# armadaproject/armada

Measured on NVIDIA H100. Metric: job-placements/sec per scheduling round; 100k nodes x 1M jobs, higher is better.
Workload: dtype int64+f64

## Files before the change

armada_b200/csrc/armada_dev.h:

```cpp
#pragma once
#include <stdint.h>
#ifndef ARMADA_EMU
#include <vector_types.h>
#endif

#include "armada_b200.h"

#define ARMADA_DEV_MAX_QUEUES 128
#define ARMADA_DEV_MAX_SLOTS 22
#define ARMADA_DEV_VARIANTS (1 + ARMADA_MAX_AWAY)

enum StatSlot {
  STAT_ITERS = 0,
  STAT_PROBES = 1,
  STAT_PLACEMENTS = 2,
  STAT_FAIR = 3,
  STAT_RESCANS = 4,
  STAT_KERNEL = 5,
  STAT_STARTUP = 6,
  STAT_RUNS = 7,
  STAT_PROF = 8,
  STAT_PROF_PQ_TOP = 8,
  STAT_PROF_GANG = 9,
  STAT_PROF_SELECT = 10,
  STAT_PROF_BIND = 11,
  STAT_BATCH_ITERS = 12,
  STAT_PROF_RESULT = 13,
  STAT_PROF_ADVANCE = 14,
  STAT_PROF_CLEAR = 15,
  STAT_BT_CYC = 16,
  STAT_BT_BUILD = 16,
  STAT_BT_HORIZON = 17,
  STAT_BT_RANK = 18,
  STAT_BT_WAIT = 19,
  STAT_BT_COMMIT = 20,
  STAT_BT_CONTROL = 21,
  STAT_BT_BATCHES = 22,
  STAT_BT_EPILOGUE = 23,
  STAT_BT_DBG = 24,
  STAT_CHAIN_BUSY = 24,
  STAT_CHAIN_WAIT = 25,
  STAT_PIPELINE_RUNS = 26,
  STAT_BT_CUT = 27,
  STAT_SLOW_STEPS = 28,
  STAT_SLOW_CYCLES = 29,
  STAT_REFILLS = 30,
  STAT_REFILL_CYCLES = 31,
  STAT_TL_PRECREATE = 32,
  STAT_TL_FIRST_BATCH_WAIT = 33,
  STAT_TL_AFTER_CHAIN_WAIT = 34,
  STAT_TL_FAILED_ITERS = 35,
  STAT_TL_FAILED_CYCLES = 36,
  STAT_TL_FAIR_QUERY = 37,
  STAT_TL_LEVEL_SCAN = 38,
  STAT_TL_EVICTED_REBIND = 39,
  STAT_GL_WAIT_INDEX = 40,
  STAT_GL_RING_FULL = 41,
  STAT_GL_SELECT_QUEUED = 42,
  STAT_GL_BIND_QUEUED = 43,
  STAT_GL_FAIR_VICTIMS = 44,
  STAT_GL_PROLOGUE = 45,
  STAT_GL_SELECT_COUNT = 46,
  STAT_GATE_RUN = 47,
  STAT_GATE_SKIPPED = 48,
  STAT_BT_FAILS = 49,
  STAT_COUNT = 50,
};

enum CountSlot {
  CNT_SCHED_JOBS = 0,
  CNT_SCHED_GANGS = 1,
  CNT_EVICTED_JOBS = 2,
  CNT_TERMINATION = 3,
  CNT_GLOBAL_TOKENS = 4,
  CNT_ERROR = 5,
  CNT_COUNT = 8,
};
#define ARMADA_DEV_E_DEADLINE 100

struct DevCfg {
  int32_t D, R, PL, PC, Q, C, T, S, rows;
  uint32_t N, J, G;
  int32_t indexed_resource[ARMADA_MAX_RESOURCES];
  int64_t res_scale[ARMADA_MAX_RESOURCES];
  int32_t key_shift[ARMADA_MAX_RESOURCES];
  int32_t res_key_shift[ARMADA_MAX_RESOURCES];
  int32_t res_key_width[ARMADA_MAX_RESOURCES];
  int32_t node_bits;
  int32_t key_total_bits;
  int32_t key_width[ARMADA_MAX_RESOURCES];
  unsigned long long key_guard;
  int32_t swar_ok;
  int32_t cls_global;
  int32_t exact;
  int64_t index_res[ARMADA_MAX_RESOURCES];
  int32_t collect_excl;
  int32_t k32_ok;
  int32_t min_bind_prio;
  int32_t priorities[ARMADA_MAX_PRIORITIES];
  ArmadaPriorityClass pcs[ARMADA_MAX_PRIORITY_CLASSES];
  int64_t total_resources[ARMADA_MAX_RESOURCES];
  double drf_mult[ARMADA_MAX_RESOURCES];
  int64_t max_to_schedule[ARMADA_MAX_RESOURCES];
  uint8_t has_round_limit, protect_uncapped, prefer_large, disable_home, disable_away, disable_gang_away,
      global_inf, _pad;
  double protected_fraction;
  uint32_t max_lookback, disallowed_mask;
  double global_tokens;
  int64_t global_burst;
  int32_t max_slots, sw, tw;
  int32_t win_w;
  uint32_t off_cls, off_win, off_touched, off_slot, off_skey, off_srow, off_ssc, off_sgpos, off_hb_key, off_hb_row, off_hb_sc,
      off_ring, off_bt_k0, off_bt_k1, off_bt_id;
  int32_t bt_wq;
  int32_t bt_np;
  uint32_t uni_V;
  uint32_t floating_mask;
  int32_t floating_configured;
  int64_t floating_limit[ARMADA_MAX_RESOURCES];
// ... 54 lines not shown
  const int64_t* queue_burst;
  const uint8_t* queue_inf;
  int64_t* alloc;
  uint32_t* bound_node;
  uint8_t* evicted_on_node;
  int32_t* sched_prio;
  uint8_t* q_successful;
  uint8_t* q_unsuccessful;
  uint8_t* q_rescheduled;
  uint8_t* q_evicted;
  uint8_t* q_reason;
  uint8_t* jc_evicted;
  uint32_t* jc_card;
  uint32_t* assigned_node;
  uint8_t* in_preempted;
  uint8_t* in_scheduled;
  uint8_t* in_sae;
  uint8_t* ev_mark;
  uint8_t* gang_ev;
  uint8_t* has_pctx;
  uint32_t* res_node;
  int32_t* res_sched_at;
  int32_t* res_preempted_at;
  uint8_t* res_method;
  uint32_t* res_seq;
  uint32_t* fp_seq;
  uint8_t* fp_flags;
  uint32_t* gang_fill;
  uint32_t* gang_buf;
  int32_t* ev_index_of_job;
  uint32_t* ev_job_by_index;
  uint8_t* ev_alive;
  uint32_t* evq_start;
  uint32_t* evq_jobs;
  uint64_t* sort_keys;
  uint64_t* sort_keys2;
  uint32_t* sort_vals;
  uint32_t* sort_vals2;
  uint32_t* counters;
  uint8_t* unfeasible;
  unsigned long long* g0;
  unsigned long long* g0_tmp;
  uint32_t* g0_sc;
  uint32_t* bt_job;
  uint32_t* bt_cls;
  uint32_t* bt_pos;
  uint32_t* bt_rank;
  uint2* bt_seq;
  int64_t* bt_asum;
  uint32_t* bt_card;
  uint4* bt_item;
  uint32_t* bt_gnode;
  uint32_t* gang_bak;
  const uint32_t* gang_uni_label;
  const uint32_t* uni_start;
  const uint32_t* class_uni_row;
  const uint8_t* gang_simple;
  uint32_t* excl;
  const uint32_t* row_type_excl;
  UndoRec* undo_log;
  uint32_t* fp_head;
  uint32_t* fp_next;
  uint32_t* nl_start;
  uint2* nl_item;
  uint32_t* nl_pos;
  uint32_t* nver;
  uint32_t* fc_ver;
  uint32_t* bver;
  uint32_t* fc_bver;
  unsigned long long* fc_bmax;
  int64_t* q_alloc;
  int64_t* q_alloc_pc;
  double* q_fair;
  double* q_tokens;
  int64_t* s_scheduled;
  int64_t* s_evicted;
  int64_t* s_counts;
  uint32_t* dbg_host;
  unsigned long long* stats;
};
```

armada_b200/csrc/armada_host.inc:

```

#define CUDA_TRY(expr)                                                                     \
  do {                                                                                     \
    cudaError_t _e = (expr);                                                               \
    if (_e != cudaSuccess) {                                                               \
      g_last_error = std::string(#expr) + ": " + cudaGetErrorString(_e);                   \
      return ARMADA_E_CUDA;                                                                \
    }                                                                                      \
  } while (0)

#ifdef ARMADA_EMU
static std::recursive_mutex& emu_mutex() {
  static std::recursive_mutex m;
  return m;
}
#define ARMADA_EMU_SERIAL std::lock_guard<std::recursive_mutex> emu_lock_(emu_mutex())
#else
#define ARMADA_EMU_SERIAL ((void)0)
#endif

template <class T>
struct PinnedVec {
  T* p = nullptr;
  size_t n = 0, cap = 0;
  PinnedVec() = default;
// ... 1045 lines not shown
  DA(P.alloc, (size_t)PL * D * N);
  DA(P.xkey, cfg.exact ? (size_t)PL * N : 1);
  DA(P.cls_glob, cfg.cls_global ? sizeof(ClassRec) * (size_t)C : 16);
  DA(P.bound_node, J);
  DA(P.evicted_on_node, J);
  DA(P.sched_prio, J);
  DA(P.q_successful, J);
  DA(P.q_unsuccessful, J);
  DA(P.q_rescheduled, J);
  DA(P.q_evicted, J);
  DA(P.q_reason, J);
  DA(P.jc_evicted, J);
  DA(P.jc_card, J);
  DA(P.assigned_node, J);
  DA(P.in_preempted, J);
  DA(P.in_scheduled, J);
  DA(P.in_sae, J);
  DA(P.ev_mark, J);
  DA(P.gang_ev, G);
  DA(P.has_pctx, J);
  DA(P.res_node, J);
  DA(P.res_sched_at, J);
  DA(P.res_preempted_at, J);
  DA(P.res_method, J);
  DA(P.res_seq, J);
  DA(P.fp_seq, J);
  DA(P.fp_flags, 4 * (size_t)J);
  DA(P.gang_fill, G);
  DA(P.gang_buf, h.gang_off[G]);
  DA(P.ev_index_of_job, J);
  DA(P.ev_job_by_index, J);
  DA(P.ev_alive, J);
  DA(P.evq_start, Q + 1);
  DA(P.evq_jobs, J);
  DA(P.sort_keys, J);
  DA(P.sort_keys2, J);
  DA(P.sort_vals, std::max(J, N));
  DA(P.sort_vals2, std::max(J, N));
  DA(P.counters, 16);
  DA(P.unfeasible, C);
  DA(P.g0, N);
  DA(P.g0_tmp, N);
  P.g0_sc = (uint32_t*)P.g0_tmp;
  DA(P.bt_job, 2 * (size_t)Q * 64);
  DA(P.bt_cls, 2 * (size_t)Q * 64);
  DA(P.bt_pos, 2 * (size_t)Q * 64);
  DA(P.bt_rank, 2 * (size_t)Q * 64);
  DA(P.bt_seq, 2 * (size_t)Q * 64);
  DA(P.bt_asum, 2 * (size_t)Q * ARMADA_MAX_RESOURCES);
  DA(P.bt_card, 2 * (size_t)Q * 64);
  DA(P.bt_item, 2 * (size_t)Q * 64);
  DA(P.bt_gnode, 2 * (size_t)Q * 64 * 64);
  DA(P.gang_bak, 32 * (4 + ARMADA_MAX_RESOURCES * 2));
  DA(P.excl, cfg.collect_excl ? (size_t)J * ARMADA_EXCLUDED_KINDS : 16);
  DA(P.undo_log, 3 * (size_t)J + 16);
  DA(P.ev_rec, J);
  DA(P.fp_head, N);
  DA(P.fp_next, J);
  DA(P.nl_start, (size_t)N + 1);
  DA(P.nl_item, J);
  DA(P.nl_pos, J);
  DA(P.nver, N);
  DA(P.fc_ver, 16 * (size_t)N);
  DA(P.bver, (N + 255) / 256 + 1);
  DA(P.fc_bver, 8 * ((size_t)(N + 255) / 256 + 1));
  DA(P.fc_bmax, 8 * ((size_t)(N + 255) / 256 + 1));
  DA(P.q_alloc, (size_t)Q * D);
  DA(P.q_alloc_pc, (size_t)Q * PC * D);
  DA(P.q_fair, (size_t)Q * 3);
  DA(P.q_tokens, Q);
  DA(P.s_scheduled, D);
  DA(P.s_evicted, D);
  DA(P.s_counts, CNT_COUNT);
  DA(P.stats, STAT_COUNT);
  {
    void* dp = nullptr;
    CUDA_TRY(cudaHostGetDevicePointer(&dp, r->h_dbg, 0));
    P.dbg_host = (uint32_t*)dp;
  }
  DA(r->d_state, J);
  DA(r->d_method, J);
  DA(r->d_reason, J);
  DA(r->d_node, J);
  DA(r->d_sched_at, J);
  DA(r->d_preempted_at, J);
  DA(r->d_evict_queue, Q);
  DA(r->d_oversub, N);
  DA(r->d_hist, 256 * (size_t)grid_for(std::max<uint32_t>(std::max(J, N), 1), RS_THREADS * RS_ITEMS) + 1024);
  if (!in->queue_allocated_by_pc || !in->queue_constrained_demand) {
    int64_t* d_demand_pc = nullptr;
    DA(d_demand_pc, (size_t)Q * PC * D);
    CUDA_TRY(cudaMemsetAsync(d_demand_pc, 0, (size_t)Q * PC * D * sizeof(int64_t), r->stream));
    ARMADA_LAUNCH(k_snapshot_jobs, grid_for(std::max<uint32_t>(J, 1)), 256, 0, r->stream, cfg, P, const_cast<int64_t*>(P.queue_alloc_pc0), d_demand_pc,
                  in->queue_allocated_by_pc ? 0 : 1);
    if (!in->queue_constrained_demand) {
      ARMADA_LAUNCH(k_snapshot_queues, grid_for((size_t)Q * D, 128), 128, 0, r->stream, cfg, P, d_demand_pc, const_cast<int64_t*>(P.queue_cdemand));
    }
    CUDA_TRY(cudaGetLastError());
  }
#undef DA
  CUDA_TRY(cudaStreamSynchronize(r->stream));
  return ARMADA_OK;
}
#undef UNSUP
#undef PINNED
}
// ... 234 lines not shown
  const ArmadaRound::Snapshot& h = r->snap;
  if (!r->uploaded || !h.valid) return fail_status(ARMADA_E_STATE, "armada_round_download_snapshot without armada_round_upload_cluster");
  auto out = [](auto* dst, const auto& src) {
    if (dst) std::copy(src.begin(), src.end(), dst);
  };
  out(node_state, h.state);
  out(node_allocatable, h.alloc);
  out(node_static_class, h.sclass);
  out(total_resources, h.total);
  out(max_resources_to_schedule, h.max_to_schedule);
  out(queue_limit, h.queue_limit);
  return ARMADA_OK;
}

#define ROUND_LAUNCH(r, kern, grid, block, smem, ...) \
  do { ARMADA_LAUNCH(kern, grid, block, smem, (r)->stream, __VA_ARGS__); ++(r)->launches; } while (0)

static void radix_sort(ArmadaRound* r, uint32_t n, const std::vector<int>& shifts, unsigned long long*& keys, unsigned long long*& keys_tmp,
                       uint32_t*& vals, uint32_t*& vals_tmp) {
  const uint32_t blocks = grid_for(n, RS_THREADS * RS_ITEMS);
  for (int shift : shifts) {
    ROUND_LAUNCH(r, k_rs_hist, blocks, RS_THREADS, 0, keys, n, shift, r->d_hist);
    ROUND_LAUNCH(r, k_rs_scan, 1, 1024, 0, r->d_hist, 256 * blocks);
    ROUND_LAUNCH(r, k_rs_scatter, blocks, RS_THREADS, 0, keys, vals, keys_tmp, vals_tmp, n, shift, r->d_hist);
    std::swap(keys, keys_tmp);
    std::swap(vals, vals_tmp);
  }
}

static int32_t sort_evicted(ArmadaRound* r, uint32_t n) {
  DevCfg& c = r->cfg;
  DevPtrs& P = r->P;
  unsigned long long *k0 = (unsigned long long*)P.sort_keys, *k1 = (unsigned long long*)P.sort_keys2;
  uint32_t *v0 = P.sort_vals, *v1 = P.sort_vals2;
  if (n > 0) {
    int rank_bytes = (bits_for(c.J > 1 ? c.J - 1 : 1) + 7) / 8;
    std::vector<int> shifts;
    for (int b = 0; b < rank_bytes; ++b) shifts.push_back(8 * b);
    int queue_bytes = (bits_for(c.Q > 1 ? (uint32_t)c.Q - 1 : 1) + 7) / 8;
    for (int b = 0; b < queue_bytes; ++b) shifts.push_back(32 + 8 * b);
    radix_sort(r, n, shifts, k0, k1, v0, v1);
    ROUND_LAUNCH(r, k_copy_u32, grid_for(n), 256, 0, P.evq_jobs, v0, n);
    ROUND_LAUNCH(r, k_build_ev_records, grid_for(n), 256, 0, c, P, n);
  }
  ROUND_LAUNCH(r, k_evq_bounds, grid_for((size_t)c.Q + 1, 128), 128, 0, c, P, k0, n);
  CUDA_TRY(cudaGetLastError());
  return ARMADA_OK;
}

static int32_t sort_g0(ArmadaRound* r) {
  DevCfg& c = r->cfg;
  DevPtrs& P = r->P;
  const uint32_t n = c.N;
  ROUND_LAUNCH(r, k_g0_keys, grid_for(n), 256, 0, c, P);
  unsigned long long *k0 = P.g0, *k1 = P.g0_tmp;
  uint32_t *v0 = P.sort_vals, *v1 = P.sort_vals2;
  std::vector<int> shifts;
  for (int shift = 0; shift < r->key_bits; shift += 8) shifts.push_back(shift);
  radix_sort(r, n, shifts, k0, k1, v0, v1);
  if (shifts.size() & 1) {
    CUDA_TRY(cudaMemcpyAsync(P.g0, P.g0_tmp, (size_t)n * sizeof(unsigned long long), cudaMemcpyDeviceToDevice, r->stream));
  }
  ROUND_LAUNCH(r, k_g0_sc, grid_for(n), 256, 0, c, P);
#ifdef ARMADA_EMU
  if (getenv("EMU_DUMP_G0")) {
    fprintf(stderr, "g0 (N=%u node_bits=%d key_bits=%d shifts", n, c.node_bits, r->key_bits);
    for (int i = 0; i < c.R; ++i) fprintf(stderr, " %d", c.key_shift[i]);
    fprintf(stderr, "):");
    for (uint32_t i = 0; i < n; ++i) fprintf(stderr, " %llx", P.g0[i]);
    fprintf(stderr, "\n");
  }
#endif
  CUDA_TRY(cudaGetLastError());
  return ARMADA_OK;
}

static void launch_xkeys(ArmadaRound* r) { ROUND_LAUNCH(r, k_xkeys, grid_for((size_t)r->cfg.PL * r->cfg.N), 256, 0, r->cfg, r->P); }

static int32_t run_reset_bind(ArmadaRound* r) {
  DevCfg& c = r->cfg;
  if (c.collect_excl) CUDA_TRY(cudaMemsetAsync(r->P.excl, 0, (size_t)c.J * ARMADA_EXCLUDED_KINDS * sizeof(uint32_t), r->stream));
  ROUND_LAUNCH(r, k_reset, r->num_sms * 4, 256, 0, c, r->P);
  ROUND_LAUNCH(r, k_bind_running, grid_for(std::max<uint32_t>(c.J, 1)), 256, 0, c, r->P);
  ROUND_LAUNCH(r, k_queue_init, 1, 32, 0, c, r->P);
  return ARMADA_OK;
}

static int32_t run_evict(ArmadaRound* r, int pass, uint32_t* evicted) {
  DevCfg& c = r->cfg;
  DevPtrs& P = r->P;
  const uint32_t gj = grid_for(std::max<uint32_t>(c.J, 1)), gg = grid_for(std::max<uint32_t>(c.G, 1));
  if (pass == 1) {
    ROUND_LAUNCH(r, k_evict_queue_flags, grid_for(c.Q, 128), 128, 0, c, P, r->d_evict_queue);
    ROUND_LAUNCH(r, k_evict_balance, gj, 256, 0, c, P, r->d_evict_queue);
  } else {
    CUDA_TRY(cudaMemsetAsync(P.counters, 0, sizeof(uint32_t), r->stream));
    ROUND_LAUNCH(r, k_oversub_mask, grid_for(c.N), 256, 0, c, P, r->d_oversub);
    ROUND_LAUNCH(r, k_evict_oversub, gj, 256, 0, c, P, r->d_oversub);
  }
  ROUND_LAUNCH(r, k_evict_gangs, gj, 256, 0, c, P);
  ROUND_LAUNCH(r, k_evict_account, gj, 256, 0, c, P, pass);
  ROUND_LAUNCH(r, k_clear_gang_ev, gg, 256, 0, c, P);
  CUDA_TRY(cudaMemcpyAsync(evicted, P.counters, sizeof(uint32_t), cudaMemcpyDeviceToHost, r->stream));
  CUDA_TRY(cudaStreamSynchronize(r->stream));
  return ARMADA_OK;
}
// ... 9 lines not shown
  a.with_queued = pass == 1;
  a.skip_key_check = pass == 2;
  a.consider_priority = pass == 2;
  a.assign_indices = pass == 2 || num_evicted > 0;
  a.pass = pass;
  a.num_evicted = num_evicted;
  a.budget_ns = budget_ns;
  a.g0_valid = pass == 1 && !r->cfg.exact;
  const PassKernel kern = pass_kernel(r->cfg.D);
  CUDA_TRY(cudaEventRecord(r->evp[2 * pass - 2], r->stream));
  ROUND_LAUNCH(r, kern, 1, PASS_THREADS, r->smem_bytes, r->cfg, r->P, a);
  CUDA_TRY(cudaEventRecord(r->evp[2 * pass - 1], r->stream));
  return ARMADA_OK;
}

static int32_t snapshot_first_pass(ArmadaRound* r) {
  DevPtrs& P = r->P;
  cudaStream_t s = r->stream;
  const size_t Jn = r->cfg.J;
  CUDA_TRY(cudaMemcpyAsync(P.fp_seq, P.res_seq, Jn * sizeof(uint32_t), cudaMemcpyDeviceToDevice, s));
  const uint8_t* flags[4] = {P.q_successful, P.q_rescheduled, P.q_unsuccessful, P.q_reason};
  for (int k = 0; k < 4; ++k) CUDA_TRY(cudaMemcpyAsync(P.fp_flags + k * Jn, flags[k], Jn, cudaMemcpyDeviceToDevice, s));
  return ARMADA_OK;
}

static int32_t run_finalize(ArmadaRound* r) {
  ROUND_LAUNCH(r, k_finalize, grid_for(std::max<uint32_t>(r->cfg.J, 1)), 256, 0, r->cfg, r->P, r->d_state, r->d_node, r->d_sched_at,
               r->d_preempted_at, r->d_method, r->d_reason);
  CUDA_TRY(cudaEventRecord(r->ev1, r->stream));
  CUDA_TRY(cudaGetLastError());
  cudaError_t e = cudaStreamSynchronize(r->stream);
  if (e != cudaSuccess) {
    g_last_error = std::string("cudaStreamSynchronize: ") + cudaGetErrorString(e) + watchdog_report(r->h_dbg);
    return ARMADA_E_CUDA;
  }
  return ARMADA_OK;
}

static int32_t read_stats(ArmadaRound* r, uint32_t e1, uint32_t e2) {
  long long counts[CNT_COUNT];
  unsigned long long dstats[STAT_COUNT];
  CUDA_TRY(cudaMemcpy(counts, r->P.s_counts, sizeof(counts), cudaMemcpyDeviceToHost));
  CUDA_TRY(cudaMemcpy(dstats, r->P.stats, sizeof(dstats), cudaMemcpyDeviceToHost));
  if (counts[CNT_ERROR] == ARMADA_DEV_E_DEADLINE)
    return fail_status(ARMADA_E_DEADLINE, "the round did not finish within its time budget; nothing was committed");
  if (counts[CNT_ERROR] != 0) return fail_status(ARMADA_E_INTERNAL, "device invariant violated, code " + std::to_string(counts[CNT_ERROR]));
  float ms = 0;
  CUDA_TRY(cudaEventElapsedTime(&ms, r->ev0, r->ev1));
  r->stats = ArmadaRoundStats{};
  if (getenv("ARMADA_PRINT_STATS"))
    fprintf(stderr,
            "armada stats: kernel_cycles=%llu startup=%llu pipeline_runs=%llu chain_busy=%llu chain_wait=%llu epilogue=%llu precreate=%llu first_batch_wait=%llu "
            "after_chain_wait=%llu failed_iters=%llu failed_cycles=%llu fair_query_cycles=%llu level_scan_cycles=%llu evicted_rebind_cycles=%llu "
            "gate_scans=%llu gate_skips=%llu bt_fails=%llu\n",
            dstats[STAT_KERNEL], dstats[STAT_STARTUP], dstats[STAT_RUNS], dstats[STAT_CHAIN_BUSY], dstats[STAT_CHAIN_WAIT], dstats[STAT_BT_EPILOGUE],
            dstats[STAT_TL_PRECREATE], dstats[STAT_TL_FIRST_BATCH_WAIT], dstats[STAT_TL_AFTER_CHAIN_WAIT], dstats[STAT_TL_FAILED_ITERS],
            dstats[STAT_TL_FAILED_CYCLES], dstats[STAT_TL_FAIR_QUERY], dstats[STAT_TL_LEVEL_SCAN], dstats[STAT_TL_EVICTED_REBIND],
            dstats[STAT_GATE_RUN], dstats[STAT_GATE_SKIPPED], dstats[STAT_BT_FAILS]);
  if (getenv("ARMADA_PRINT_STATS"))
    fprintf(stderr,
            "armada general loop: wait_index_warps=%llu ring_full=%llu select_queued=%llu (n=%llu) bind_queued=%llu fair_victims=%llu iteration_prologue=%llu\n",
            dstats[STAT_GL_WAIT_INDEX], dstats[STAT_GL_RING_FULL], dstats[STAT_GL_SELECT_QUEUED], dstats[STAT_GL_SELECT_COUNT],
            dstats[STAT_GL_BIND_QUEUED], dstats[STAT_GL_FAIR_VICTIMS], dstats[STAT_GL_PROLOGUE]);
  r->stats.loop_iterations = dstats[STAT_ITERS];
  r->stats.probes = dstats[STAT_PROBES];
  r->stats.placements = dstats[STAT_PLACEMENTS];
  r->stats.fair_preemption_scans = dstats[STAT_FAIR];
  r->stats.tree_rescans = dstats[STAT_RESCANS];
  for (int i = 0; i < 8; ++i) r->stats.phase_cycles[i] = dstats[STAT_PROF + i];
  for (int i = 0; i < 8; ++i) r->stats.batch_cycles[i] = dstats[STAT_BT_CYC + i];
  for (int i = 0; i < 8; ++i) r->stats.batch_debug[i] = dstats[STAT_BT_DBG + i];
  r->stats.evicted_pass1 = e1;
  r->stats.evicted_pass2 = e2;
  r->stats.gpu_launches = r->launches;
  r->stats.device_ms = ms;
  float p1 = 0, p2 = 0;
  CUDA_TRY(cudaEventElapsedTime(&p1, r->evp[0], r->evp[1]));
  if (e2 > 0) CUDA_TRY(cudaEventElapsedTime(&p2, r->evp[2], r->evp[3]));
  r->stats.schedule_pass_ms = p1 + p2;
  return ARMADA_OK;
}

int32_t armada_round_run(ArmadaRound* r, ArmadaRoundStats* stats) { return armada_round_run_deadline(r, stats, 0); }

int32_t armada_round_run_deadline(ArmadaRound* r, ArmadaRoundStats* stats, uint64_t budget_ns) {
  if (!r) return fail_status(ARMADA_E_INVALID, "null handle");
  const auto t_run0 = std::chrono::steady_clock::now();
  auto budget_left = [&]() -> unsigned long long {
    if (!budget_ns) return 0ull;
    const uint64_t used = (uint64_t)std::chrono::duration_cast<std::chrono::nanoseconds>(std::chrono::steady_clock::now() - t_run0).count();
    return used >= budget_ns ? 1ull : (unsigned long long)(budget_ns - used);
  };
  if (!r->uploaded) return fail_status(ARMADA_E_STATE, "armada_round_run before armada_round_upload");
  ARMADA_EMU_SERIAL;
  CUDA_TRY(cudaSetDevice(r->device));
  r->launches = 0;
  CUDA_TRY(cudaEventRecord(r->ev0, r->stream));
  int32_t st;
  uint32_t e1 = 0, e2 = 0;
  if ((st = run_reset_bind(r)) || (st = run_evict(r, 1, &e1)) || (st = sort_evicted(r, e1))) return st;
  const unsigned long long budget1 = budget_left();
  if ((st = build_index(r, 1)) || (st = run_pass(r, 1, e1, budget1)) || (st = snapshot_first_pass(r))) return st;
  if ((st = run_evict(r, 2, &e2))) return st;
  if (e2 > 0) {
    if ((st = sort_evicted(r, e2))) return st;
    const unsigned long long budget2 = budget_left();
    if ((st = build_index(r, 2)) || (st = run_pass(r, 2, e2, budget2))) return st;
  }
  if ((st = run_finalize(r)) || (st = read_stats(r, e1, e2))) return st;
  if (stats) *stats = r->stats;
  r->ran = true;
// ... 374 lines not shown
```

armada_b200/csrc/armada_pass.inc:

```

#define g_c (H->env_c)
#define g_p (H->env_p)
#define g_a (H->env_a)

#define PASS_WARPS 16
#define PASS_THREADS (PASS_WARPS * 32)
#define IDX_WARPS 15
#define CTL_WARP (PASS_WARPS - 1)
#define IDX_OWNERS (IDX_WARPS - 1)
#define WIN 32
#define WIN_TARGET 12
#define WIN_LOW 4
#define MSG_CAP 32
#define TLOG_CAP 32

enum { MSG_EXIT = 0, MSG_UPDATE0 = 1, MSG_NEWSLOT = 2, MSG_SCAN = 3, MSG_BATCH = 4, MSG_SUCC = 5, MSG_FAIR = 6 };
#define BT_RING 32

#define REC_EVICTED 0x80000000u
#define REC_GANG 0x40000000u
#define REC_QEV 0x20000000u
#define REC_GS 0x10000000u
#define REC_GSL 0x08000000u
#define REC_CLS_MASK 0x00FFFFFFu
// ... 3013 lines not shown
#pragma unroll
    for (int t = 0; t < ARMADA_DEV_MAX_SLOTS; ++t) Df[t] = 0;
    const unsigned long long G = g_c.key_guard;
    const uint32_t okm = H->slot_okp;
    uint32_t seen = 0;
    for (uint32_t pos = (uint32_t)w * 32u + (uint32_t)l; pos < g_c.N; pos += IDX_WARPS * 32u) {
      const unsigned long long gk = g_p.g0[pos];
      const uint32_t n = (uint32_t)(gk & nodemask);
      if ((V.touched[n >> 5] >> (n & 31)) & 1u) continue;
      if ((gk >> g_c.key_total_bits) != 0) continue;
      const uint32_t sc = g_p.g0_sc[pos];
      uint32_t m = 0;
#pragma unroll
      for (int t = 0; t < ARMADA_DEV_MAX_SLOTS; ++t)
        if (t < ns) {
          const SlotHdr& sh = V.slot[t];
          const bool f = sh.active && ((okm >> t) & 1u) && Idx<DMAX>::slot_static(sh, sc) && ((((gk | G) - H->slot_preq[t]) & G) == G);
          m |= (f ? 1u : 0u) << t;
        }
#pragma unroll
      for (int t = 0; t < ARMADA_DEV_MAX_SLOTS; ++t) Df[t] |= ((m >> t) & 1u) ? ~m : m;
      uint32_t fresh = m & ~seen;
      seen |= m;
      while (fresh) {
        const int t = __ffs(fresh) - 1;
        fresh &= fresh - 1;
        atomicMin(&H->grp_first[t], pos);
      }
    }
#pragma unroll
    for (int t = 0; t < ARMADA_DEV_MAX_SLOTS; ++t)
      if (t < ns) {
        const uint32_t r = __reduce_or_sync(FULL, Df[t]);
        if (l == 0 && r) atomicOr(&H->grp_diff[t], r);
      }
    __threadfence_block();
    bar_idx();
    if (w == 0) {
      if (l < ns && V.slot[l].active) {
        uint32_t leader = (uint32_t)l;
        for (int t = 0; t < l; ++t)
          if (V.slot[t].active && V.slot[t].row == V.slot[l].row && !((H->grp_diff[l] >> t) & 1u)) {
            leader = (uint32_t)t;
            break;
          }
        H->grp_of[l] = leader;
      }
      if (l == 0) H->grp_ns = ns;
    }
    __threadfence_block();
    bar_idx();
  }

  static __device__ ARMADA_NOINLINE void fill_lazy(int w, bool have_first) {
    const int ns = H->num_slots;
    if (w < IDX_OWNERS)
      for (int s = w; s < ns; s += IDX_OWNERS) {
        SlotHdr& sh = V.slot[s];
        if (!sh.active || !sh.lazy) continue;
        const uint32_t first = have_first ? H->grp_first[s] : 0u;
        __syncwarp();
        if (lane_id() == 0) {
          if (have_first && sh.cursor < first) {
            const uint32_t c = first < g_c.N ? first : g_c.N;
            sh.cursor = c;
            sh.wm = c < g_c.N ? g_p.g0[c] : KEY_INF;
          }
          sh.lazy = 0;
        }
        __syncwarp();
        Idx<DMAX>::ensure_head(s, true);
      }
    __threadfence_block();
    bar_idx();
  }

  static __device__ ARMADA_NOINLINE void table_build() {
    const int l = lane_id();
    const int ns = H->num_slots;
    const uint32_t ltm = (1u << l) - 1u;
    bool valid = false;
    uint32_t node = NONE;
    bool ok = true;
    BtRes* T = H->bt_ring;
    for (int s = 0; s < ns && ok; ++s) {
      const SlotHdr& sh = V.slot[s];
      if (!sh.active) continue;
      if (sh.lostmin != KEY_INF) ok = false;
      const uint32_t cnt = sh.cnt;
      const bool tch = (uint32_t)l < cnt && V.sgpos[s * WIN + l] == NONE;
      const uint32_t nid = tch ? (uint32_t)(V.skey[s * WIN + l] & nodemask) : NONE;
      if (!__ballot_sync(FULL, tch)) continue;
      bool dupe = false;
#pragma unroll
      for (int j = 0; j < 32; ++j) {
        const uint32_t nj = __shfl_sync(FULL, node, j);
        dupe = dupe || (tch && nj == nid);
      }
      const uint32_t newm = __ballot_sync(FULL, tch && !dupe);
      if (!newm) continue;
      const uint32_t freem = ~__ballot_sync(FULL, valid);
      const int nnew = __popc(newm);
      if (nnew > __popc(freem)) {
        ok = false;
        break;
      }
// ... 369 lines not shown
    return 1;
  }

  static __device__ __forceinline__ uint32_t warp_min_u32(uint32_t v) {
#ifdef ARMADA_EMU
    return __reduce_min_sync(FULL, v);
#else
    uint32_t m;
    asm volatile("redux.sync.min.u32 %0, %1, 0xffffffff;" : "=r"(m) : "r"(v));
    return m;
#endif
  }
  template <bool K32, class KT>
  static __device__ __forceinline__ int place(Lane<K32>& X, uint32_t& have, const uint32_t exh, const uint32_t lead, const KT Gk, const uint4 r, uint4* recp) {
    bool win, cand;
    uint32_t sbit;
    if (K32) {
      sbit = r.y;
      const uint32_t d = (uint32_t)X.Y - r.x;
      const bool fit = ((d & (uint32_t)Gk) == (uint32_t)Gk) && (X.mystat & sbit);
      const uint32_t m = warp_min_u32(fit ? X.ck : 0xFFFFFFFFu);
      if (m == 0xFFFFFFFFu) return 2;
      win = X.ck == m;
      cand = m & 1u;
      if (win) {
        X.Y = d;
        X.ck -= r.w;
        recp->w = X.node;
      }
    } else {
      sbit = r.w;
      const unsigned long long d = (unsigned long long)X.Y - (((unsigned long long)r.y << 32) | r.x);
      const bool fit = ((d & (unsigned long long)Gk) == (unsigned long long)Gk) && (X.mystat & sbit);
      const unsigned long long m = warp_min_u64(fit ? (unsigned long long)X.Y : KEY_INF);
      if (m == KEY_INF) return 2;
      win = (unsigned long long)X.Y == m;
      cand = m & 1ull;
      if (win) {
        X.Y = d;
        recp->w = X.node;
      }
    }
    if (cand) {
      if (win) {
        if (K32) X.ck &= ~1u;
        else X.Y &= ~(KT)1;
        X.mystat = X.fullstat;
        atomicOr(&V.touched[X.node >> 5], 1u << (X.node & 31));
      }
      have = exh | __reduce_or_sync(FULL, is_cand<K32>(X) ? X.mystat : 0u);
      if (~have & lead) return 3;
    }
    return 0;
  }
  template <bool K32, class KT>
  static __device__ __forceinline__ int place_pair(Lane<K32>& X, uint32_t& have, const uint32_t exh, const uint32_t lead, const KT Gk, uint4* const rec,
                                                   uint32_t& t, const uint32_t total) {
    const KT NOFIT = ~(KT)0;
    auto req_of = [](const uint4 r) -> KT { return K32 ? (KT)r.x : (KT)(((unsigned long long)r.y << 32) | r.x); };
    auto grp_of = [](const uint4 r) -> uint32_t { return K32 ? r.y : r.w; };
    auto wmin = [](const KT v) -> KT { return K32 ? (KT)warp_min_u32((uint32_t)v) : (KT)warp_min_u64((unsigned long long)v); };
    auto gfit = [Gk](const KT d) -> bool { return (~d & Gk) == 0; };
    auto row_won = [](const KT d) -> KT { return K32 ? d : (KT)(d & ~(KT)1); };
    uint4 ra = rec[t], rb = rec[t + 1];
    for (;;) {
      const uint32_t left = total - t;
      const uint4 ran = rec[t + 2];
      uint4 rbn = rb;
      if (left >= 2) rbn = rec[t + 3];
      const KT ck = K32 ? (KT)X.ck : X.Y;
      const uint32_t sw = ((K32 ? X.ck : (uint32_t)X.Y) & 1u) ? X.fullstat : X.mystat;
      const KT da = X.Y - req_of(ra), db = X.Y - req_of(rb);
      const KT Ya = row_won(da), cka = K32 ? (KT)((X.ck - ra.w) & ~1u) : Ya;
      const KT dab = Ya - req_of(rb);
      const KT ka = (X.mystat & grp_of(ra)) ? ck : NOFIT;
      const KT ma = wmin(gfit(da) ? ka : NOFIT);
      const KT kb0 = (gfit(db) && (X.mystat & grp_of(rb))) ? ck : NOFIT;
      const KT kb1 = (gfit(dab) && (sw & grp_of(rb))) ? cka : NOFIT;
      const bool wa = ck == ma;
      const KT mb = wmin(wa ? kb1 : kb0);
      if (ma == NOFIT) return 2;
      const KT cka_post = wa ? cka : ck;
      const KT Yb = wa ? row_won(dab) : row_won(db);
      const KT ckb = K32 ? (KT)(((uint32_t)cka_post - rb.w) & ~1u) : Yb;
      if (wa) {
        X.Y = Ya;
        if (K32) X.ck = (uint32_t)cka;
        X.mystat = sw;
        rec[t].w = X.node;
      }
      ++t;
      if (ma & 1u) {
        if (wa) atomicOr(&V.touched[X.node >> 5], 1u << (X.node & 31));
        have = exh | __reduce_or_sync(FULL, is_cand<K32>(X) ? X.mystat : 0u);
        if (~have & lead) return 3;
      }
      if (t == total) return 0;
      if (mb == NOFIT) return 2;
      const bool wb = cka_post == mb;
      if (wb) {
        X.Y = Yb;
        if (K32) X.ck = (uint32_t)ckb;
        X.mystat = sw;
        rec[t].w = X.node;
      }
      ++t;
      if (mb & 1u) {
        if (wb) atomicOr(&V.touched[X.node >> 5], 1u << (X.node & 31));
        have = exh | __reduce_or_sync(FULL, is_cand<K32>(X) ? X.mystat : 0u);
        if (~have & lead) return 3;
      }
      if (t == total) return 0;
      ra = ran;
      rb = rbn;
    }
  }
  template <bool K32, class KT>
  static __device__ __forceinline__ bool ensure_groups(Lane<K32>& X, uint32_t& have, uint32_t& exh, const uint32_t lead, int ns, const KT Gk) {
    uint32_t need = ~have & lead;
    while (need) {
      const uint32_t s = (uint32_t)(__ffs(need) - 1);
      int r = install_bulk<K32, KT>(X, have, s, ns, Gk);
      if (r == 0) {
        if (!window_refill(s)) {
          have |= 1u << s;
          exh |= 1u << s;
          r = 1;
        } else {
          r = install_bulk<K32, KT>(X, have, s, ns, Gk);
        }
      }
      if (r != 1 && !install_general<K32>(&X, &have, &exh, s, ns)) return false;
      need = ~have & lead;
    }
    return true;
  }

  static __device__ __forceinline__ void chain_wait_first() {
    SPIN_BEGIN;
    while (Idx<DMAX>::uniform_ld(&H->pl_ready) == 0) {
      Ctl<DMAX>::service_fence();
      SPIN_CHECK(20);
      armada_emu_yield();
    }
    __threadfence_block();
  }

  static __device__ __forceinline__ long long chain_wait_batch(uint32_t kb) {
    const long long tw0 = clock64();
    SPIN_BEGIN;
    while ((uint32_t)Idx<DMAX>::uniform_ld(&H->pl_ready) <= kb) {
      SPIN_CHECK(21);
      armada_emu_yield();
    }
    __threadfence_block();
    return clock64() - tw0;
  }

  static __device__ __forceinline__ void chain_hand_over(uint32_t kb, uint32_t t, uint32_t total, bool failed) {
    __threadfence_block();
    __syncwarp();
    if (lane_id() == 0) {
      H->bt_done[kb & 1u] = t;
// ... 572 lines not shown
#define BT_CLOCK(slot)                                  \
  do {                                                  \
    if (w == 0 && lane_id() == 0) {                     \
      long long _t = clock64();                         \
      H->stat[slot] += (unsigned long long)(_t - t0);   \
      t0 = _t;                                          \
    }                                                   \
  } while (0)
  static __device__ __forceinline__ void produce(int w, int b, bool first, long long& t0) {
    for (int q = w; q < g_c.Q; q += IDX_WARPS) batch_build(q, b, first);
    __threadfence_block();
    bar_idx();
    BT_CLOCK(STAT_BT_BUILD);
    if (w == 0) {
      batch_horizon(b);
      if (lane_id() == 0) H->pl_skip = first ? 0u : ld_vol(&H->pl_cut);
    }
    __threadfence_block();
    bar_idx();
    BT_CLOCK(STAT_BT_HORIZON);
    if (H->pl_skip) return;
    batch_rank(w, b);
    for (int q = w; q < g_c.Q; q += IDX_WARPS) batch_advance(q, b);
    __threadfence();
    bar_idx();
    BT_CLOCK(STAT_BT_RANK);
  }

  static __device__ ARMADA_NOINLINE void restart(int w, int b, long long& t0) {
    const uint4 tail = __ldcg(&g_p.bt_item[buf_of(b).goff + H->bt_done[b] - 1]);
    const uint2 job = __ldcg(&g_p.bt_seq[buf_of(b).goff + H->bt_done[b] - 1]);
    const int qf = (int)tail.x;
    for (int q = w; q < g_c.Q; q += IDX_WARPS)
      if (H->bt_repeek[q] && q != qf) Ctl<DMAX>::pq_update(q, true);
    __threadfence_block();
    bar_idx();
    if (w == 0) {
      Ctl<DMAX>::mark_unfeasible(job.y, ARMADA_REASON_JOB_DOES_NOT_FIT);
      Ctl<DMAX>::pq_update(qf, true);
      if (lane_id() < g_c.D) H->sp_sched[lane_id()] = H->s_scheduled[lane_id()];
      if (lane_id() == 0) st_vol(&H->pl_cut, 0u);
    }
    __threadfence_block();
    bar_idx();
    produce(w, b, true, t0);
  }

  static __device__ ARMADA_NOINLINE void batch_run(int w) {
    long long t0 = clock64();
    const int ns = H->num_slots;
    const bool regroup = g_c.swar_ok && H->grp_ns != ns;
    if (regroup) group_slots(w);
    fill_lazy(w, regroup);
    produce(w, 0, true, t0);
    if (w == 0) table_build();
    __threadfence_block();
    bar_idx();
    const bool run = H->bt_total[0] > 0;
    if (run && w < IDX_OWNERS)
      for (int s = w; s < ns; s += IDX_OWNERS)
        if (V.slot[s].active) win_strip(s, false);
    __threadfence_block();
    bar_idx();
    if (w == 0 && lane_id() == 0) st_vol(&H->pl_ready, 1u);
    uint32_t kb = 0;
    while (H->bt_total[kb & 1u] > 0) {
      const int b = (int)(kb & 1u);
      produce(w, b ^ 1, false, t0);
      if (w == 0 && lane_id() == 0) st_vol(&H->pl_ready, kb + 2u);
      {
        SPIN_BEGIN;
        while ((uint32_t)Idx<DMAX>::uniform_ld(&H->pl_chain) <= kb) {
          SPIN_CHECK(22);
          idle_pause();
        }
        __threadfence_block();
      }
      BT_CLOCK(STAT_BT_WAIT);
      apply_results(w, b);
      for (int q = w; q < g_c.Q; q += IDX_WARPS) batch_commit(q, b);
      __threadfence();
      bar_idx();
      if (w == 0 && lane_id() == 0) {
        H->pl_seq += H->bt_done[b];
        H->stat[STAT_BT_BATCHES] += 1;
        if (H->bt_done[b] < H->bt_total[b]) H->stat[STAT_BT_CUT] += 1;
      }
      BT_CLOCK(STAT_BT_COMMIT);
      if (H->bt_fail[b]) {
        restart(w, b, t0);
        if (w == 0 && lane_id() == 0) st_vol(&H->pl_ready, kb + 3u);
        kb += 2;
        continue;
      }
      if (H->bt_done[b] < H->bt_total[b]) break;
      ++kb;
    }
    {
      SPIN_BEGIN;
      while (Idx<DMAX>::uniform_ld(&H->pl_home) == 0) {
        SPIN_CHECK(23);
        idle_pause();
      }
      __threadfence_block();
    }
    if (run && w < IDX_OWNERS)
// ... 173 lines not shown
```

armada_b200/csrc/armada_round.cu:

```cuda
#ifdef ARMADA_EMU
#include "cuda_emu.h"
#else
#include <cuda_runtime.h>
#define ARMADA_LAUNCH(kern, grid, block, smem, stream, ...) kern<<<(grid), (block), (smem), (stream)>>>(__VA_ARGS__)
#define ARMADA_DYN_SMEM(name) extern __shared__ __align__(16) unsigned char name[]
#define ARMADA_NAMED_BARRIER(id, count) asm volatile("bar.sync %0, %1;" ::"n"(id), "n"(count) : "memory")
static __device__ __forceinline__ void armada_emu_yield() {}
#define ARMADA_NOINLINE __noinline__
#define ARMADA_EMU_MARK(id) ((void)0)
#define ARMADA_PREFETCH_L1(p) asm volatile("prefetch.global.L1 [%0];" ::"l"(p))
#endif

#include <algorithm>
#include <atomic>
#include <memory>
#include <condition_variable>
#include <mutex>
#include <chrono>
#include <thread>
#include <type_traits>
#include <cmath>
#include <cstdio>
#include <cstring>
#include <numeric>
// ... 321 lines not shown
    tmp[threadIdx.x] = v;
    __syncthreads();
    for (int off = 1; off < 1024; off <<= 1) {
      uint32_t t = threadIdx.x >= (unsigned)off ? tmp[threadIdx.x - off] : 0;
      __syncthreads();
      tmp[threadIdx.x] += t;
      __syncthreads();
    }
    uint32_t incl = tmp[threadIdx.x];
    if (i < len) hist[i] = carry + incl - v;
    __syncthreads();
    if (threadIdx.x == 1023) carry += incl;
    __syncthreads();
  }
}
__global__ void k_rs_scatter(const unsigned long long* keys, const uint32_t* vals, unsigned long long* keys_out,
                             uint32_t* vals_out, uint32_t n, int shift, const uint32_t* hist) {
  __shared__ unsigned long long sk[RS_THREADS * RS_ITEMS];
  __shared__ uint32_t sv[RS_THREADS * RS_ITEMS];
  size_t base = (size_t)blockIdx.x * RS_THREADS * RS_ITEMS;
  uint32_t cnt = 0;
  for (int i = 0; i < RS_ITEMS; ++i) {
    size_t k = base + (size_t)i * RS_THREADS + threadIdx.x;
    uint32_t li = i * RS_THREADS + threadIdx.x;
    if (k < n) {
      sk[li] = keys[k];
      sv[li] = vals[k];
    }
  }
  __syncthreads();
  uint32_t m = n - base < (size_t)RS_THREADS * RS_ITEMS ? (uint32_t)(n - base) : RS_THREADS * RS_ITEMS;
  uint32_t off = hist[(size_t)threadIdx.x * gridDim.x + blockIdx.x];
  for (uint32_t li = 0; li < m; ++li) {
    if (((sk[li] >> shift) & 255) == threadIdx.x) {
      keys_out[off + cnt] = sk[li];
      vals_out[off + cnt] = sv[li];
      ++cnt;
    }
  }
}

__global__ void k_g0_keys(DevCfg c, DevPtrs P) {
  size_t n = blockIdx.x * (size_t)blockDim.x + threadIdx.x;
  if (n >= c.N) return;
  unsigned long long key = n;
  bool neg = false;
  for (int i = 0; i < c.R; ++i) {
    int64_t v = P.alloc[(size_t)c.indexed_resource[i] * c.N + n];
    neg = neg || v < 0;
    key |= (unsigned long long)v << c.key_shift[i];
  }
  unsigned long long marker = 1ull << c.key_total_bits;
  P.g0[n] = neg ? (marker | n) : key;
}

__device__ __forceinline__ unsigned long long xfield_of(int64_t v, int64_t res) {
  if (v < 0) return 0ull;
  long long q = (long long)((double)v / (double)res);
  while (q * res > v) --q;
  while ((q + 1) * res <= v) ++q;
  return (unsigned long long)q + 1ull;
}
__global__ void k_xkeys(DevCfg c, DevPtrs P) {
  size_t i = blockIdx.x * (size_t)blockDim.x + threadIdx.x;
  if (i >= (size_t)c.PL * c.N) return;
  const size_t p = i / c.N, n = i - p * c.N;
  unsigned long long key = P.node_xrank[n];
  for (int k = 0; k < c.R; ++k)
    key |= xfield_of(P.alloc[(p * c.D + c.indexed_resource[k]) * c.N + n], c.index_res[k]) << c.key_shift[k];
  P.xkey[i] = key;
}

__global__ void k_snapshot_jobs(DevCfg c, DevPtrs P, int64_t* alloc_pc, int64_t* demand_pc, int want_alloc) {
  size_t j = blockIdx.x * (size_t)blockDim.x + threadIdx.x;
  if (j >= c.J) return;
  const uint32_t q = P.job_queue[j];
  if (q == NONE) return;
  const uint32_t cls = P.job_class[j];
  const uint32_t pc = P.class_pc[cls];
  const bool running = P.job_node0[j] != NONE;
  const bool cordoned = P.queue_cordoned[q] != 0;
  for (int d = 0; d < c.D; ++d) {
    const int64_t r = P.class_req_raw[(size_t)cls * c.D + d];
    if (!r) continue;
    if (running && want_alloc) atomic_add_i64(&alloc_pc[((size_t)q * c.PC + pc) * c.D + d], r);
    if (running || !cordoned) atomic_add_i64(&demand_pc[((size_t)q * c.PC + pc) * c.D + d], r);
  }
}
__global__ void k_snapshot_queues(DevCfg c, DevPtrs P, const int64_t* demand_pc, int64_t* cdemand) {
  int i = blockIdx.x * blockDim.x + threadIdx.x;
  if (i >= c.Q * c.D) return;
  const int q = i / c.D, d = i - q * c.D;
  int64_t sum = 0;
  for (int pc = 0; pc < c.PC; ++pc) {
    int64_t v = demand_pc[((size_t)q * c.PC + pc) * c.D + d];
    if (P.queue_has_limit[(size_t)q * c.PC + pc]) {
      const int64_t lim = P.queue_limit[((size_t)q * c.PC + pc) * c.D + d];
      if (lim < v) v = lim;
    }
    sum += v;
  }
  cdemand[i] = sum;
}

__global__ void k_g0_sc(DevCfg c, DevPtrs P) {
  size_t i = blockIdx.x * (size_t)blockDim.x + threadIdx.x;
// ... 89 lines not shown
```

Before: 43.66 million.

## Add supply-component analysis and skip candidate rescans when group unchanged

Adds a per-node-class max-capacity table built in the key kernel, and a warp routine that computes connected components of active slots by shared feasible supply. For now the routine only records statistics. In place_pair, the full warp OR-reduction that rebuilds the candidate mask after a win is replaced by a cheaper check that rebuilds it only when other groups were affected or the current group has no candidates left. The new component pass, the memset and the atomicMax in k_g0_keys add overhead, and the shortcut could leave the have mask stale.

```diff
diff --git a/armada_b200/csrc/armada_dev.h b/armada_b200/csrc/armada_dev.h
--- a/armada_b200/csrc/armada_dev.h
+++ b/armada_b200/csrc/armada_dev.h
@@ -64,7 +64,9 @@
   STAT_GATE_RUN = 47,
   STAT_GATE_SKIPPED = 48,
   STAT_BT_FAILS = 49,
-  STAT_COUNT = 50,
+  STAT_BT_COMPONENTS = 50,
+  STAT_BT_SPLIT_RUNS = 51,
+  STAT_COUNT = 52,
 };
 
 enum CountSlot {
@@ -225,6 +227,7 @@
   uint4* bt_item;
   uint32_t* bt_gnode;
   uint32_t* gang_bak;
+  int64_t* sc_max;
   const uint32_t* gang_uni_label;
   const uint32_t* uni_start;
   const uint32_t* class_uni_row;
diff --git a/armada_b200/csrc/armada_host.inc b/armada_b200/csrc/armada_host.inc
--- a/armada_b200/csrc/armada_host.inc
+++ b/armada_b200/csrc/armada_host.inc
@@ -1121,6 +1121,7 @@
   DA(P.bt_item, 2 * (size_t)Q * 64);
   DA(P.bt_gnode, 2 * (size_t)Q * 64 * 64);
   DA(P.gang_bak, 32 * (4 + ARMADA_MAX_RESOURCES * 2));
+  DA(P.sc_max, (size_t)std::max(cfg.S, 1) * D);
   DA(P.excl, cfg.collect_excl ? (size_t)J * ARMADA_EXCLUDED_KINDS : 16);
   DA(P.undo_log, 3 * (size_t)J + 16);
   DA(P.ev_rec, J);
@@ -1461,6 +1462,7 @@
   DevCfg& c = r->cfg;
   DevPtrs& P = r->P;
   const uint32_t n = c.N;
+  CUDA_TRY(cudaMemsetAsync(P.sc_max, 0, (size_t)c.S * c.D * sizeof(int64_t), r->stream));
   ROUND_LAUNCH(r, k_g0_keys, grid_for(n), 256, 0, c, P);
   unsigned long long *k0 = P.g0, *k1 = P.g0_tmp;
   uint32_t *v0 = P.sort_vals, *v1 = P.sort_vals2;
@@ -1576,11 +1578,11 @@
     fprintf(stderr,
             "armada stats: kernel_cycles=%llu startup=%llu pipeline_runs=%llu chain_busy=%llu chain_wait=%llu epilogue=%llu precreate=%llu first_batch_wait=%llu "
             "after_chain_wait=%llu failed_iters=%llu failed_cycles=%llu fair_query_cycles=%llu level_scan_cycles=%llu evicted_rebind_cycles=%llu "
-            "gate_scans=%llu gate_skips=%llu bt_fails=%llu\n",
+            "gate_scans=%llu gate_skips=%llu bt_fails=%llu supply_components=%llu split_runs=%llu\n",
             dstats[STAT_KERNEL], dstats[STAT_STARTUP], dstats[STAT_RUNS], dstats[STAT_CHAIN_BUSY], dstats[STAT_CHAIN_WAIT], dstats[STAT_BT_EPILOGUE],
             dstats[STAT_TL_PRECREATE], dstats[STAT_TL_FIRST_BATCH_WAIT], dstats[STAT_TL_AFTER_CHAIN_WAIT], dstats[STAT_TL_FAILED_ITERS],
             dstats[STAT_TL_FAILED_CYCLES], dstats[STAT_TL_FAIR_QUERY], dstats[STAT_TL_LEVEL_SCAN], dstats[STAT_TL_EVICTED_REBIND],
-            dstats[STAT_GATE_RUN], dstats[STAT_GATE_SKIPPED], dstats[STAT_BT_FAILS]);
+            dstats[STAT_GATE_RUN], dstats[STAT_GATE_SKIPPED], dstats[STAT_BT_FAILS], dstats[STAT_BT_COMPONENTS], dstats[STAT_BT_SPLIT_RUNS]);
   if (getenv("ARMADA_PRINT_STATS"))
     fprintf(stderr,
             "armada general loop: wait_index_warps=%llu ring_full=%llu select_queued=%llu (n=%llu) bind_queued=%llu fair_victims=%llu iteration_prologue=%llu\n",
diff --git a/armada_b200/csrc/armada_pass.inc b/armada_b200/csrc/armada_pass.inc
--- a/armada_b200/csrc/armada_pass.inc
+++ b/armada_b200/csrc/armada_pass.inc
@@ -3089,6 +3089,61 @@
     bar_idx();
   }
 
+  static __device__ ARMADA_NOINLINE void supply_components() {
+    const int l = lane_id();
+    const int ns = H->num_slots;
+    const bool act = l < ns && V.slot[l].active;
+    const uint32_t actm = __ballot_sync(FULL, act);
+    uint32_t adj = act ? 1u << l : 0u;
+    if (g_a.g0_valid) {
+      for (int s0 = 0; s0 < g_c.S; s0 += 32) {
+        const int s = s0 + l;
+        uint32_t m = 0;
+        if (s < g_c.S)
+          for (int t = 0; t < ns; ++t) {
+            if (!((actm >> t) & 1u) || !Idx<DMAX>::slot_static(V.slot[t], (uint32_t)s)) continue;
+            bool f = true;
+            for (int d = 0; d < g_c.D; ++d) f = f && g_p.sc_max[(size_t)s * g_c.D + d] >= V.slot[t].req[d];
+            if (f) m |= 1u << t;
+          }
+        for (int j = 0; j < 32; ++j) {
+          const uint32_t mj = __shfl_sync(FULL, m, j);
+          if ((mj >> l) & 1u) adj |= mj;
+        }
+      }
+      if (g_c.swar_ok) {
+        const uint32_t ld = act ? (H->grp_of[l] & 31u) : 32u;
+        if (act) adj |= 1u << ld;
+        for (int j = 0; j < 32; ++j)
+          if (__shfl_sync(FULL, ld, j) == (uint32_t)l) adj |= 1u << j;
+      }
+      uint32_t away = 0;
+      if (!g_c.disable_away)
+        for (int c = l; c < g_c.C; c += 32) {
+          const ClassRec& k = V.cls[c];
+          if (k.slot[0] >= 0 && k.row[1] != NONE) away |= 1u << k.slot[0];
+        }
+      away = __reduce_or_sync(FULL, away) & actm;
+      if ((away >> l) & 1u) adj |= away;
+    } else {
+      adj = act ? actm : 0u;
+    }
+    for (int it = 0; it < 5; ++it) {
+      uint32_t m = adj;
+      for (int j = 0; j < 32; ++j) {
+        const uint32_t aj = __shfl_sync(FULL, adj, j);
+        if ((adj >> j) & 1u) m |= aj;
+      }
+      adj = m;
+    }
+    const uint32_t nc = (uint32_t)__popc(__ballot_sync(FULL, act && __ffs(adj) - 1 == l));
+    if (l == 0) {
+      H->stat[STAT_BT_COMPONENTS] += nc;
+      if (nc > 1) H->stat[STAT_BT_SPLIT_RUNS] += 1;
+    }
+    __syncwarp();
+  }
+
   static __device__ ARMADA_NOINLINE void fill_lazy(int w, bool have_first) {
     const int ns = H->num_slots;
     if (w < IDX_OWNERS)
@@ -3564,6 +3619,15 @@
       if (~have & lead) return 3;
     }
     return 0;
+  }
+  template <bool K32>
+  static __device__ __forceinline__ bool cand_left(const Lane<K32>& X, uint32_t& have, const uint32_t exh, const uint32_t lead, const uint32_t g,
+                                                   const uint32_t mold) {
+    const bool more = __any_sync(FULL, (mold & ~g) != 0u);
+    const bool left = __any_sync(FULL, is_cand<K32>(X) && (X.mystat & g) != 0u);
+    if (more) have = exh | __reduce_or_sync(FULL, is_cand<K32>(X) ? X.mystat : 0u);
+    else if (!left) have = (have & ~g) | exh;
+    return (~have & lead) == 0u;
   }
   template <bool K32, class KT>
   static __device__ __forceinline__ int place_pair(Lane<K32>& X, uint32_t& have, const uint32_t exh, const uint32_t lead, const KT Gk, uint4* const rec,
@@ -3595,6 +3659,7 @@
       const KT cka_post = wa ? cka : ck;
       const KT Yb = wa ? row_won(dab) : row_won(db);
       const KT ckb = K32 ? (KT)(((uint32_t)cka_post - rb.w) & ~1u) : Yb;
+      const uint32_t mold_a = wa ? X.mystat : 0u;
       if (wa) {
         X.Y = Ya;
         if (K32) X.ck = (uint32_t)cka;
@@ -3604,12 +3669,12 @@
       ++t;
       if (ma & 1u) {
         if (wa) atomicOr(&V.touched[X.node >> 5], 1u << (X.node & 31));
-        have = exh | __reduce_or_sync(FULL, is_cand<K32>(X) ? X.mystat : 0u);
-        if (~have & lead) return 3;
+        if (!cand_left<K32>(X, have, exh, lead, grp_of(ra), mold_a)) return 3;
       }
       if (t == total) return 0;
       if (mb == NOFIT) return 2;
       const bool wb = cka_post == mb;
+      const uint32_t mold_b = wb ? X.mystat : 0u;
       if (wb) {
         X.Y = Yb;
         if (K32) X.ck = (uint32_t)ckb;
@@ -3619,8 +3684,7 @@
       ++t;
       if (mb & 1u) {
         if (wb) atomicOr(&V.touched[X.node >> 5], 1u << (X.node & 31));
-        have = exh | __reduce_or_sync(FULL, is_cand<K32>(X) ? X.mystat : 0u);
-        if (~have & lead) return 3;
+        if (!cand_left<K32>(X, have, exh, lead, grp_of(rb), mold_b)) return 3;
       }
       if (t == total) return 0;
       ra = ran;
@@ -4299,6 +4363,7 @@
     const bool regroup = g_c.swar_ok && H->grp_ns != ns;
     if (regroup) group_slots(w);
     fill_lazy(w, regroup);
+    if (w == 0) supply_components();
     produce(w, 0, true, t0);
     if (w == 0) table_build();
     __threadfence_block();
diff --git a/armada_b200/csrc/armada_round.cu b/armada_b200/csrc/armada_round.cu
--- a/armada_b200/csrc/armada_round.cu
+++ b/armada_b200/csrc/armada_round.cu
@@ -397,6 +397,12 @@
   }
   unsigned long long marker = 1ull << c.key_total_bits;
   P.g0[n] = neg ? (marker | n) : key;
+  const uint32_t s = P.node_sclass[n];
+  for (int d = 0; d < c.D; ++d) {
+    const int64_t v = P.node_total[(size_t)d * c.N + n];
+    long long* m = reinterpret_cast<long long*>(&P.sc_max[(size_t)s * c.D + d]);
+    if (v > *(volatile long long*)m) atomicMax(m, (long long)v);
+  }
 }
 
 __device__ __forceinline__ unsigned long long xfield_of(int64_t v, int64_t res) {
```

Result: no change. 43.27 million (median of 6 runs) (-0.9%).
